# SEAME-pt/Team02-ObjectDetection

Measured on AMD Instinct MI355X. Metric: images/sec fwd+bwd MobileNetV2UNet 256x512 bs=32/GPU, higher is better.
Workload: dtype f32; 1 GPU; MobileNetV2UNet 10-class fwd+bwd+Adam, 256x512, bs=32/GPU (BASELINE configs[1]); model=MobileNetV2UNet, global_batch=32, parallelism=dp1, collectives=RCCL (torch.distributed nccl), optimizer=seg_amd.Adam (HIP, one launch)

## Files before the change

### include/segamd.h

```cpp
#ifndef SEGAMD_H
#define SEGAMD_H
#include <hip/hip_runtime.h>
#include <stdint.h>
#ifdef __cplusplus
extern "C" {
#endif



int seg_conv_igemm(const float* in, long ldin, int N, int H, int W, int Cin,
                   const float* wk, int ldk, const float* bias,
                   float* out, long ldout, int Ho, int Wo, int Cout,
                   int ks, int stride, int pad,
                   const float* add, long ldadd, float* stat, hipStream_t stream);
int seg_conv_igemm_act(const float* in, long ldin, int N, int H, int W, int Cin,
                       const float* wk, int ldk, const float* bias,
                       float* out, long ldout, int Ho, int Wo, int Cout,
                       int ks, int stride, int pad,
                       const float* add, long ldadd, float* stat, int act, float* work, int splits,
                       hipStream_t stream);
int seg_conv_igemm_bf16(const float* in, long ldin, int N, int H, int W, int Cin,
                        const float* wk, int ldk, const float* bias,
                        float* out, long ldout, int Ho, int Wo, int Cout,
                        int ks, int stride, int pad,
// ... 2 lines not shown
int seg_conv_igemm_f16(const float* in, long ldin, int N, int H, int W, int Cin,
                       const float* wk, int ldk, const float* bias,
                       float* out, long ldout, int Ho, int Wo, int Cout,
                       int ks, int stride, int pad,
                       const float* add, long ldadd, float* stat, int act, float* work, int splits,
                       hipStream_t stream);
int seg_conv_pw_row_tiles(long M);
int seg_conv_pw(const float* in, long ldin, long M, int K, const float* wk, int ldk, const float* bias,
                float* out, long ldout, int N, const float* add, long ldadd, float* stat,
                const float* in_scale, const float* in_shift, int in_act, hipStream_t stream);
int seg_conv_igemm_splits(long M, int Cout, int Cin, int ks);
int seg_conv_igemm_tiles(long M, int Cout);
int seg_conv_igemm_plan_b1(long M, int Cout, int Cin, int ks, int* out);
int seg_conv_igemm_act_ic(const float* in, long ldin, int N, int H, int W, int Cin, const float* wk, int ldk,
                          const float* bias, float* out, long ldout, int Ho, int Wo, int Cout, int ks, int stride,
                          int pad, const float* add, long ldadd, int act, float* work, int splits, int tile, unsigned* cnt,
                          hipStream_t stream);
int seg_conv_igemm_bf16_ic(const float* in, long ldin, int N, int H, int W, int Cin, const float* wk, int ldk,
                           const float* bias, float* out, long ldout, int Ho, int Wo, int Cout, int ks, int stride,
                           int pad, const float* add, long ldadd, int act, float* work, int splits, int tile, unsigned* cnt,
                           hipStream_t stream);
int seg_conv_igemm_f16_ic(const float* in, long ldin, int N, int H, int W, int Cin, const float* wk, int ldk,
                          const float* bias, float* out, long ldout, int Ho, int Wo, int Cout, int ks, int stride,
                          int pad, const float* add, long ldadd, int act, float* work, int splits, int tile, unsigned* cnt,
                          hipStream_t stream);

int seg_conv_igemm_bnout_ok(long M, int Cout, int bf16);
int seg_conv_igemm_bnout(const float* in, long ldin, int N, int H, int W, int Cin, const float* wk, int ldk,
                         float* out, long ldout, int Cout, int ks, const float* add, long ldadd,
                         const float* by, long ldby, const float* bscale, const float* bshift,
                         const float* bmean, int bact, float* bpart, hipStream_t stream);

int seg_igemm_force_tile(int t);
int seg_conv_igemm_tile(long M, int Cout);
int seg_conv_igemm_row_tiles(long M, int Cout, int* tile_rows);

int seg_pack_conv_weight(const float* w, float* wk, int Cout, int Cin, int ks, int ldk,
                         int mode, int kin_pad, hipStream_t stream);

int seg_conv_wgrad_splits(long M, int Cout, int Cin, int ks);
int seg_conv_wgrad_splits_bf16(long M, int Cout, int Cin, int ks);
int seg_conv_wgrad(const float* dy, long lddy, const float* x, long ldx,
                   int N, int H, int W, int Cin, int Ho, int Wo, int Cout,
                   int ks, int stride, int pad, float* part, int splits, hipStream_t stream);

int seg_conv_wgrad_bf16(const float* dy, long lddy, const float* x, long ldx,
                        int N, int H, int W, int Cin, int Ho, int Wo, int Cout,
                        int ks, int stride, int pad, float* part, int splits, hipStream_t stream);

int seg_conv_igemm_xf(const float* in, long ldin, int N, int H, int W, int Cin,
                      const float* wk, int ldk, const float* bias,
                      float* out, long ldout, int Ho, int Wo, int Cout,
                      int ks, int stride, int pad,
                      const float* add, long ldadd, float* stat, const float* in_scale, const float* in_shift,
                      int in_act, hipStream_t stream);
int seg_conv_igemm_bf16_xf(const float* in, long ldin, int N, int H, int W, int Cin,
                           const float* wk, int ldk, const float* bias,
                           float* out, long ldout, int Ho, int Wo, int Cout,
                           int ks, int stride, int pad,
                           const float* add, long ldadd, float* stat, const float* in_scale, const float* in_shift,
                           int in_act, hipStream_t stream);
int seg_conv_wgrad_xf(const float* dy, long lddy, const float* x, long ldx,
                      int N, int H, int W, int Cin, int Ho, int Wo, int Cout,
                      int ks, int stride, int pad, float* part, int splits,
                      const float* in_scale, const float* in_shift, int in_act, hipStream_t stream);
int seg_conv_wgrad_bf16_xf(const float* dy, long lddy, const float* x, long ldx,
                           int N, int H, int W, int Cin, int Ho, int Wo, int Cout,
                           int ks, int stride, int pad, float* part, int splits,
                           const float* in_scale, const float* in_shift, int in_act, hipStream_t stream);

int seg_conv_wgrad_reduce(const float* part, int splits, float* dw, int Cout, int Cin, int ks,
                          int mode, int accumulate, hipStream_t stream);

int seg_conv_wino_pick(int N, int H, int W, int Cin, int Cout);
int seg_conv_wino_tile_rows(void);
int seg_conv_wino_row_tiles(int N, int H, int W);
int seg_conv_wino(const float* in, long ldin, int N, int H, int W, int Cin, const float* wk, int ldk,
                  const float* bias, float* out, long ldout, int Cout, const float* add, long ldadd,
                  float* stat, float* work, hipStream_t stream);
int seg_conv_wino_fused(const float* in, long ldin, int N, int H, int W, int Cin, const float* wk, int ldk,
                        const float* bias, float* out, long ldout, int Cout, const float* add, long ldadd, float* stat,
                        hipStream_t stream);
int seg_conv_wino_fused_ok(int N, int H, int W, long ldin);
int seg_conv_wino_wgrad_pick(int N, int H, int W, int Cin, int Cout);
int seg_conv_wino_wgrad_splits(int N, int H, int W, int Cin, int Cout);
int seg_conv_wino_wgrad(const float* dy, long lddy, const float* x, long ldx, int N, int H, int W, int Cin,
                        int Cout, float* part, int splits, hipStream_t stream);
int seg_conv_wino_wgrad16_splits(int N, int H, int W, int Cin, int Cout);
int seg_conv_wino_wgrad16(const float* dy, long lddy, const float* x, long ldx, int N, int H, int W, int Cin,
                          int Cout, float* part, int splits, hipStream_t stream);
int seg_conv_wino_wgrad_reduce(float* part, int splits, float* dw, int Cout, int Cin, int Cin_pad,
                               int accumulate, hipStream_t stream);

int seg_conv_halo_ok(int N, int H, int W, int Cin, int Cout);
int seg_conv_halo_pick(int N, int H, int W, int Cin, int Cout);
int seg_conv_halo_row_tiles(int N, int H, int W);
int seg_conv_halo(const float* in, long ldin, int N, int H, int W, int Cin, const float* wk, int ldk,
                  const float* bias, float* out, long ldout, int Cout, const float* add, long ldadd,
                  float* stat, hipStream_t stream);

typedef struct seg_pack_job {
  const float* w;
  float* wk;
  int cout, cin, ks, ldk, mode, kin_pad;
  int blk0, nblk;
} seg_pack_job;
int seg_pack_batch(const void* jobs, int njobs, long nblocks, hipStream_t stream);

int seg_pack_dw_weight(const float* w, float* wk, int C, hipStream_t stream);
int seg_dw_fwd(const float* in, long ldin, int N, int H, int W, int C,
               const float* in_scale, const float* in_shift, int in_act, const float* wk,
               float* out, long ldout, int Ho, int Wo, int stride, hipStream_t stream);
int seg_dw_fwd_bias_act(const float* in, long ldin, int N, int H, int W, int C, const float* wk,
                        const float* bias, int act, float* out, long ldout, int Ho, int Wo, int stride,
                        hipStream_t stream);
int seg_dw_dgrad(const float* dy, long lddy, int N, int Ho, int Wo, int C, const float* wk,
                 float* dx, long lddx, int H, int W, int stride, int accumulate, hipStream_t stream);
long seg_dw_wgrad_blocks(int N, int Ho, int Wo, int C);
int seg_dw_wgrad(const float* dy, long lddy, const float* x, long ldx, int N, int H, int W, int C,
                 const float* in_scale, const float* in_shift, int in_act,
                 int Ho, int Wo, int stride, float* part, hipStream_t stream);

int seg_nchw_to_nhwc(const float* x, int N, int C, int H, int W, float* out, int ld, hipStream_t stream);

long seg_chan_workspace_floats(long M, int C);
int seg_bn_stats(const float* y, long ldy, long M, int C, const float* gamma, const float* beta,
                 float eps, float momentum, float* running_mean, float* running_var,
                 long long* num_batches_tracked, float* work,
                 float* mean, float* invstd, float* scale, float* shift, hipStream_t stream);
int seg_bn_stats_tiles(const float* part, int ntiles, int tile_rows, long M, int C, const float* gamma,
                       const float* beta, float eps, float momentum, float* running_mean, float* running_var,
                       long long* num_batches_tracked, float* mean, float* invstd, float* scale, float* shift,
                       hipStream_t stream);
long seg_bn_stats_tiles_work_floats(int ntiles, int C);
int seg_bn_stats_tiles_ws(const float* part, int ntiles, int tile_rows, long M, int C, const float* gamma,
                          const float* beta, float eps, float momentum, float* running_mean, float* running_var,
                          long long* num_batches_tracked, float* mean, float* invstd, float* scale, float* shift,
                          float* work, hipStream_t stream);
int seg_bn_eval_coef(const float* gamma, const float* beta, const float* running_mean,
                     const float* running_var, float eps, int C, float* scale, float* shift,
                     hipStream_t stream);
int seg_bn_apply(const float* y, long ldy, long M, int C, const float* scale, const float* shift,
                 int act, const float* res, long ldres, float* out, long ldout, hipStream_t stream);
int seg_bn_backward(const float* da, long ldda, const float* y, long ldy, long M, int C,
                    const float* gamma, const float* mean, const float* invstd,
                    const float* scale, const float* shift, int act,
                    float* dgamma, float* dbeta, float* work, float* dy, long lddy, hipStream_t stream);
int seg_bn_bwd_finalize_tiles(const float* part, int ntiles, long M, int C, const float* gamma,
                              const float* invstd, float* dgamma, float* dbeta, float* coef, hipStream_t stream);
int seg_bn_bwd_coef(const float* da, long ldda, const float* y, long ldy, long M, int C, const float* gamma,
                    const float* mean, const float* invstd, const float* scale, const float* shift, int act,
                    float* dgamma, float* dbeta, float* work, float* coef, hipStream_t stream);
int seg_bn_bwd_apply(const float* da, long ldda, const float* y, long ldy, long M, int C, const float* mean,
                     const float* scale, const float* shift, int act, const float* coef, float* dy, long lddy,
                     hipStream_t stream);
int seg_bn_eval_backward(const float* da, long ldda, const float* y, long ldy, long M, int C,
                         const float* scale, const float* shift, int act, float* dy, long lddy,
                         hipStream_t stream);
int seg_bn_frozen_backward(const float* da, long ldda, const float* y, long ldy, long M, int C,
                           const float* scale, const float* shift, const float* running_mean,
                           const float* running_var, float eps, int act, float* dgamma, float* dbeta,
                           float* work, float* dy, long lddy, hipStream_t stream);
int seg_colsum(const float* y, long ldy, long M, int C, float* work, float* out, int accumulate,
               hipStream_t stream);
int seg_add(const float* a, long lda, const float* b, long ldb, long M, int C, float* out, long ldout,
            hipStream_t stream);
// ... 271 lines not shown
```

### team02-objectdetection_amd/csrc/wino.hip

```cpp
#include "common.h"

#ifndef SEG_WINO_OUT_CSPLIT
#define SEG_WINO_OUT_CSPLIT 1
#endif

#ifndef SEG_WINO_OUT_QT
#define SEG_WINO_OUT_QT 4
#endif

namespace {

constexpr int kWinoQT = SEG_WINO_OUT_QT;
__device__ __attribute__((aligned(16))) float g_wzero4[4];

struct WinoArgs {
  const float* in; long ldin;
  const float* wk; int ldk;
  float* m;
  int N, H, W, Cin, Cout;
  int T, th, tw;
};

__device__ __forceinline__ void bt_row(int r, int& p0, int& p1, float& s0, float& s1) {
  p0 = r == 0 ? 0 : 1;
// ... 186 lines not shown
        for (int x = 0; x < 16; ++x) qv[x] = ld4(m + x * TC + (long)tile[q] * Cout + c);
        f32x4 r0[4], r1[4];
#pragma unroll
        for (int j = 0; j < 4; ++j) {
          r0[j] = qv[j] + qv[4 + j] + qv[8 + j];
          r1[j] = qv[4 + j] - qv[8 + j] - qv[12 + j];
        }
        y[q][0] = r0[0] + r0[1] + r0[2] + b;
        y[q][1] = r0[1] - r0[2] - r0[3] + b;
        y[q][2] = r1[0] + r1[1] + r1[2] + b;
        y[q][3] = r1[1] - r1[2] - r1[3] + b;
#pragma unroll
        for (int p = 0; p < 4; ++p) {
          if (add) y[q][p] += ld4(add + pix[q][p] * ldadd + c);
          st4(out + pix[q][p] * ldout + c, y[q][p]);
        }
      } else {
#pragma unroll
        for (int p = 0; p < 4; ++p) y[q][p] = f32x4{0.f, 0.f, 0.f, 0.f};
      }
    }
#if SEG_WINO_OUT_CSPLIT
    if (!stat) return;
#else
    if (!stat) continue;
#endif
#pragma unroll
    for (int pass = 0; pass < 2; ++pass) {
      f32x4 s = {0.f, 0.f, 0.f, 0.f};
      const f32x4 mu = pass ? bmean[cl] : f32x4{0.f, 0.f, 0.f, 0.f};
#pragma unroll
      for (int q = 0; q < QT; ++q)
        if (tok[q] && cok) {
#pragma unroll
          for (int p = 0; p < 4; ++p) {
            const f32x4 d = y[q][p] - mu;
            s += pass ? d * d : d;
          }
        }
#pragma unroll
      for (int o = 16; o < 64; o <<= 1)
#pragma unroll
        for (int j = 0; j < 4; ++j) s[j] += __shfl_xor(s[j], o, 64);
      if ((t & 63) < 16) red[wave][cl] = s;
      __syncthreads();
      if (t < 16) {
        const f32x4 tot = red[0][t] + red[1][t] + red[2][t] + red[3][t];
        const int cc = cgb + t * 4;
        if (pass == 0) bmean[t] = tot / cnt;
        if (cc < Cout) {
          float* dst = stat + ((long)blockIdx.x * 2 + pass) * Cout + cc;
#pragma unroll
          for (int j = 0; j < 4; ++j) dst[j] = tot[j];
        }
      }
      __syncthreads();
    }
  }
}

template <int BM, int BN, int WM, int WN, int NT = 256>
void launch_wino(const WinoArgs& a, hipStream_t s) {
  dim3 grid(seg_cdiv(a.T, BM) * seg_cdiv(a.Cout, BN), 1, 16);
  hipLaunchKernelGGL((wino_gemm_kernel<BM, BN, WM, WN, 32, NT>), grid, dim3(NT), 0, s, a);
}
#ifndef SEG_WINO_WIDE_MINBLK
#define SEG_WINO_WIDE_MINBLK 0
#endif
#ifndef SEG_WINO_WIDE
#define SEG_WINO_WIDE 256
#endif

struct WinoFusedArgs {
  const float* in; long ldin;
  const float* wk; int ldk;
  const float* bias;
  const float* add; long ldadd;
  float* out; long ldout;
  float* stat;
  int N, H, W, Cin, Cout;
  int T, th, tw;
  long in_elems;
  unsigned wk_bytes;
};

#ifndef SEG_WF_EXP
#define SEG_WF_EXP 0
#endif
constexpr int kFusedKC = 8;
constexpr int kFusedUR = kFusedKC + 4;
constexpr unsigned kFusedOOB = 0x80000000u;

__device__ __forceinline__ __amdgpu_buffer_rsrc_t seg_rsrc(const void* p, unsigned bytes) {
  const unsigned long v = (unsigned long)p;
  const unsigned lo = __builtin_amdgcn_readfirstlane((unsigned)v), hi = __builtin_amdgcn_readfirstlane((unsigned)(v >> 32));
  return __builtin_amdgcn_make_buffer_rsrc(reinterpret_cast<void*>(((unsigned long)hi << 32) | lo), 0,
                                           (int)__builtin_amdgcn_readfirstlane(bytes), 0x00020000);
}
__device__ __forceinline__ f32x4 seg_bld4(__amdgpu_buffer_rsrc_t r, unsigned off) {
  typedef unsigned u32x4 __attribute__((ext_vector_type(4)));
  return __builtin_bit_cast(f32x4, __builtin_amdgcn_raw_buffer_load_b128(r, off, 0, 0));
}

template <int WT>
__global__ __launch_bounds__(256) void wino_fused_kernel(WinoFusedArgs a) {
  constexpr int WN = 4 / WT, BT = 32 * WT, BC = 32 * WN;
  static_assert(WT == 2 || WT == 4, "a BN row tile (64 tiles) lies in one block");
  static_assert(16 * kWinoQT == 64, "wino_fused_kernel's BN row tile is 64 Winograd tiles");
  constexpr int USZ = 16 * BC * kFusedUR;
  constexpr int UPT = 16 * BC * (kFusedKC / 4) / 256;
  __shared__ __attribute__((aligned(16))) float Us[2 * USZ];
  __shared__ float red[4][32];

  const int tid = threadIdx.x, lane = tid & 63, wave = tid >> 6;
  const int wt = wave / WN, wn = wave % WN;
  const int row = lane & 31, h = lane >> 5;
  const int tiles_n = (a.Cout + BC - 1) / BC;
  const int lid = xcd_swizzle(blockIdx.x, gridDim.x);
  const int tn = lid % tiles_n, tm = lid / tiles_n;
  const int m0 = tm * BT, n0 = tn * BC;
  const int nfirst = m0 / (a.th * a.tw);
  const long boff = (long)nfirst * a.H * a.W * a.ldin;
  const __amdgpu_buffer_rsrc_t rin = seg_rsrc(a.in + boff, (unsigned)min((a.in_elems - boff) * 4, (long)kFusedOOB - 16));
  const __amdgpu_buffer_rsrc_t rwk = seg_rsrc(a.wk, a.wk_bytes);

  const int t = m0 + wt * 32 + row;
  const bool tok = t < a.T;
  unsigned pm = 0, pbase = 0;
  int opix = 0;
  {
    const int tt = tok ? t : 0;
    const int n = tt / (a.th * a.tw), r = tt - n * a.th * a.tw;
    const int ty = r / a.tw, tx = r - ty * a.tw;
    const int h0 = 2 * ty - 1, w0 = 2 * tx - 1;
#pragma unroll
    for (int p = 0; p < 4; ++p)
#pragma unroll
      for (int q = 0; q < 4; ++q)
        if (tok && (unsigned)(h0 + p) < (unsigned)a.H && (unsigned)(w0 + q) < (unsigned)a.W) pm |= 1u << (p * 4 + q);
    pbase = (unsigned)((((long)(n - nfirst) * a.H + h0) * a.W + w0) * a.ldin * 4) + 16u * h;
    opix = (n * a.H + 2 * ty) * a.W + 2 * tx;
  }
  const unsigned rstep = (unsigned)(a.W * a.ldin * 4), cstep = (unsigned)(a.ldin * 4);

  auto load_patch = [&](int c0, f32x4 (&d)[16]) {
    const bool cok = c0 + 4 * h < a.Cin;
    const unsigned b = pbase + 4u * c0;
#pragma unroll
    for (int p = 0; p < 4; ++p)
#pragma unroll
      for (int q = 0; q < 4; ++q) {
        const bool ok = cok && ((pm >> (p * 4 + q)) & 1u);
        d[p * 4 + q] = seg_bld4(rin, ok ? b + p * rstep + q * cstep : kFusedOOB);
      }
  };
  auto load_u = [&](int c0, f32x4 (&u)[UPT]) {
#pragma unroll
    for (int i = 0; i < UPT; ++i) {
      const int idx = tid + i * 256;
      const int xi = idx / (2 * BC), rem = idx - xi * (2 * BC);
      const int co = n0 + (rem >> 1), c = c0 + 4 * (rem & 1);
      const bool ok = co < a.Cout && c < a.Cin;
      u[i] = seg_bld4(rwk, ok ? (unsigned)((((long)xi * a.Cout + co) * a.ldk + c) * 4) : kFusedOOB);
    }
  };
  auto store_u = [&](float* dst, const f32x4 (&u)[UPT]) {
#pragma unroll
    for (int i = 0; i < UPT; ++i) {
      const int idx = tid + i * 256;
      const int xi = idx / (2 * BC), rem = idx - xi * (2 * BC);
      st4(dst + (xi * BC + (rem >> 1)) * kFusedUR + 4 * (rem & 1), u[i]);
    }
  };
  auto transform = [](f32x4 (&d)[16]) {
#pragma unroll
    for (int q = 0; q < 4; ++q) {
      const f32x4 d0 = d[q], d1 = d[4 + q], d2 = d[8 + q], d3 = d[12 + q];
      d[q] = d0 - d2;
      d[4 + q] = d1 + d2;
      d[8 + q] = d2 - d1;
      d[12 + q] = d1 - d3;
    }
#pragma unroll
    for (int r = 0; r < 4; ++r) {
      const f32x4 t0 = d[4 * r], t1 = d[4 * r + 1], t2 = d[4 * r + 2], t3 = d[4 * r + 3];
      d[4 * r] = t0 - t2;
      d[4 * r + 1] = t1 + t2;
      d[4 * r + 2] = t2 - t1;
      d[4 * r + 3] = t1 - t3;
    }
  };

  f32x16 acc[16];
#pragma unroll
  for (int x = 0; x < 16; ++x)
#pragma unroll
    for (int r = 0; r < 16; ++r) acc[x][r] = 0.f;

  const int nk = (a.Cin + kFusedKC - 1) / kFusedKC;
  const int urow = (wn * 32 + row) * kFusedUR + 4 * h;
  f32x4 d[16], ug[UPT];
  load_patch(0, d);
  load_u(0, ug);
  store_u(Us, ug);
  __syncthreads();
  for (int kc = 0; kc < nk; ++kc) {
    const bool more = kc + 1 < nk;
    f32x4 dn[16];
    if (more && !(SEG_WF_EXP & 1)) {
      load_patch((kc + 1) * kFusedKC, dn);
      load_u((kc + 1) * kFusedKC, ug);
    }
    if (SEG_WF_EXP & 1) {
#pragma unroll
      for (int q = 0; q < 16; ++q) dn[q] = d[q] * 0.5f;
    }
    if (!(SEG_WF_EXP & 2)) transform(d);
    const float* ub = Us + (kc & 1) * USZ + urow;
    f32x4 u[2][4];
#pragma unroll
    for (int j = 0; j < 4; ++j) u[0][j] = ld4(ub + j * BC * kFusedUR);
#pragma unroll
    for (int g = 0; g < 4; ++g) {
      if (g < 3) {
#pragma unroll
        for (int j = 0; j < 4; ++j) u[(g + 1) & 1][j] = ld4(ub + (4 * (g + 1) + j) * BC * kFusedUR);
      }
#pragma unroll
      for (int s2 = 0; s2 < 4; ++s2)
#pragma unroll
        for (int j = 0; j < 4; ++j)
          if (SEG_WF_EXP & 4)
            acc[4 * g + j][s2] += d[4 * g + j][s2] * u[g & 1][j][s2];
          else
            acc[4 * g + j] = __builtin_amdgcn_mfma_f32_32x32x2f32(d[4 * g + j][s2], u[g & 1][j][s2], acc[4 * g + j],
                                                                  0, 0, 0);
    }
    if (more) {
      store_u(Us + ((kc + 1) & 1) * USZ, ug);
#pragma unroll
      for (int q = 0; q < 16; ++q) d[q] = dn[q];
    }
    __syncthreads();
  }

  const int col = n0 + wn * 32 + row;
  const bool cok = col < a.Cout;
  const float b = (a.bias && cok) ? a.bias[col] : 0.f;
  auto tile_y = [&](int r, float (&y)[4]) {
    float q[16];
#pragma unroll
    for (int x = 0; x < 16; ++x) q[x] = acc[x][r];
    float r0[4], r1[4];
#pragma unroll
    for (int j = 0; j < 4; ++j) {
      r0[j] = q[j] + q[4 + j] + q[8 + j];
      r1[j] = q[4 + j] - q[8 + j] - q[12 + j];
    }
    y[0] = r0[0] + r0[1] + r0[2] + b;
    y[1] = r0[1] - r0[2] - r0[3] + b;
    y[2] = r1[0] + r1[1] + r1[2] + b;
    y[3] = r1[1] - r1[2] - r1[3] + b;
  };
  const int wbase = m0 + wt * 32 + 4 * h;
  float ssum = 0.f;
#pragma unroll
  for (int r = 0; r < 16; ++r) {
    const int tt = wbase + (r & 3) + 8 * (r >> 2);
    const long p0 = __shfl(opix, (r & 3) + 8 * (r >> 2) + 4 * h, 64);
    if (tt < a.T && cok) {
      float y[4];
      tile_y(r, y);
#pragma unroll
      for (int u = 0; u < 4; ++u) {
        const long pix = p0 + (u >> 1) * a.W + (u & 1);
        if (a.add) y[u] += a.add[pix * a.ldadd + col];
        a.out[pix * a.ldout + col] = y[u];
        ssum += y[u];
      }
    }
  }
  if (!a.stat) return;
  const int rtile = (m0 + (wt & ~1) * 32) / 64;
  const int ntile = min(64, a.T - rtile * 64);
  const int we = (wt & ~1) * WN + wn, wo = we + WN;
  float mean = 0.f;
#pragma unroll
  for (int pass = 0; pass < 2; ++pass) {
    float sv = ssum;
    if (pass) {
      sv = 0.f;
#pragma unroll
      for (int r = 0; r < 16; ++r) {
        const int tt = wbase + (r & 3) + 8 * (r >> 2);
        if (tt < a.T && cok) {
          float y[4];
          tile_y(r, y);
#pragma unroll
          for (int u = 0; u < 4; ++u) {
            const float dv = y[u] - mean;
            sv += dv * dv;
          }
        }
      }
    }
    sv += __shfl_xor(sv, 32, 64);
    if (h == 0) red[wave][row] = sv;
    __syncthreads();
    const float tot = red[we][row] + red[wo][row];
    if (pass == 0) mean = ntile > 0 ? tot / (4.f * (float)ntile) : 0.f;
    if ((wt & 1) == 0 && h == 0 && cok && ntile > 0) a.stat[((long)rtile * 2 + pass) * a.Cout + col] = tot;
    __syncthreads();
  }
}

struct WinoWgradArgs {
  const float* dy; long lddy;
  const float* x; long ldx;
  float* part;
  int N, H, W, Cin, Cout;
  int T, th, tw, kchunk;
};

__device__ __forceinline__ float arow(int i, int a) {
  return a == 0 ? (i == 3 ? 0.f : 1.f) : (i == 0 ? 0.f : (i == 2 || i == 3 ? -1.f : 1.f));
// ... 294 lines not shown
#pragma unroll
  for (int p = 0; p < 4; ++p) {
    float* slab = a.part + ((long)split * 16 + 4 * wave + p) * a.Cout * a.Cin;
#pragma unroll
    for (int ni = 0; ni < NI; ++ni) {
      const int col = n0 + ni * 32 + lrow;
      if (col >= a.Cin) continue;
#pragma unroll
      for (int mi = 0; mi < MI; ++mi)
#pragma unroll
        for (int e = 0; e < 16; ++e) {
          const int row = co0 + mi * 32 + (e & 3) + 8 * (e >> 2) + 4 * lh;
          if (row < a.Cout) slab[(long)row * a.Cin + col] = acc[p][mi][ni][e];
        }
    }
  }
}

__global__ __launch_bounds__(256) void wino_wgrad_fold_kernel(float* __restrict__ part, int splits, int L, long E4) {
  const long e = (long)blockIdx.x * 256 + threadIdx.x;
  if (e >= E4) return;
  const int s0 = blockIdx.y * L, s1 = min(splits, s0 + L);
  f32x4* p = reinterpret_cast<f32x4*>(part) + e;
  f32x4 acc = p[(long)s0 * E4];
#pragma unroll 8
  for (int s = s0 + 1; s < s1; ++s) acc += p[(long)s * E4];
  p[(long)s0 * E4] = acc;
}

__global__ __launch_bounds__(256) void wino_wgrad_reduce_kernel(const float* __restrict__ part, int splits, int stride,
                                                                int Cout, int Cin_pad, int Cin, float* __restrict__ dw,
                                                                int accumulate) {
  const long i = (long)blockIdx.x * 256 + threadIdx.x;
  if (i >= (long)Cout * Cin) return;
  const int co = (int)(i / Cin), ci = (int)(i - (long)co * Cin);
  const long plane = (long)Cout * Cin_pad, off = (long)co * Cin_pad + ci;
  float m[16];
#pragma unroll
  for (int x = 0; x < 16; ++x) m[x] = 0.f;
  for (int s = 0; s < splits; ++s) {
    const float* p = part + (long)s * stride * 16 * plane + off;
#pragma unroll
    for (int x = 0; x < 16; ++x) m[x] += p[x * plane];
  }
  float t[3][4];
#pragma unroll
  for (int j = 0; j < 4; ++j) {
    t[0][j] = m[j] + 0.5f * (m[4 + j] + m[8 + j]);
    t[1][j] = 0.5f * (m[4 + j] - m[8 + j]);
    t[2][j] = 0.5f * (m[4 + j] + m[8 + j]) + m[12 + j];
  }
  float* o = dw + i * 9;
#pragma unroll
  for (int y = 0; y < 3; ++y) {
    const float v[3] = {t[y][0] + 0.5f * (t[y][1] + t[y][2]), 0.5f * (t[y][1] - t[y][2]),
                        0.5f * (t[y][1] + t[y][2]) + t[y][3]};
#pragma unroll
    for (int x = 0; x < 3; ++x) o[y * 3 + x] = accumulate ? o[y * 3 + x] + v[x] : v[x];
  }
}

}

#ifndef SEG_WINO_FUSED
#define SEG_WINO_FUSED 1
#endif
static bool fused_fits(int N, int H, int W, long ldin) {
  const long tiles = (long)(H / 2) * (W / 2);
  const long imgs = std::min<long>(N, tiles > 0 ? 128 / tiles + 2 : N);
  return imgs * H * W * ldin * 4 < (long)kFusedOOB - 16;
}
SEG_API int seg_conv_wino_pick(int N, int H, int W, int Cin, int Cout) {
  if ((H & 1) || (W & 1) || (Cin & 3) || (Cout & 3) || N <= 0) return 0;
  if (Cin >= 256 && Cout >= 128) return 1;
  if (Cin >= 128 && Cout >= 128 && (Cout <= 2 * Cin || Cout >= 512)) return 1;
  const bool fits = fused_fits(N, H, W, Cin + 64);
  return (SEG_WINO_FUSED && fits && Cin >= 64 && (Cout >= 128 || (Cout >= 64 && Cin > 128 && Cin < 256))) ? 2 : 0;
}

SEG_API int seg_conv_wino_fused_ok(int N, int H, int W, long ldin) {
  return ((H & 1) || (W & 1) || N <= 0) ? 0 : (int)fused_fits(N, H, W, ldin);
}

SEG_API int seg_conv_wino_row_tiles(int N, int H, int W) {
  const long T = (long)N * (H / 2) * (W / 2);
  return (int)((T + 16 * kWinoQT - 1) / (16 * kWinoQT));
}

SEG_API int seg_conv_wino_tile_rows(void) { return 64 * kWinoQT; }

SEG_API int seg_conv_wino(const float* in, long ldin, int N, int H, int W, int Cin, const float* wk, int ldk,
                          const float* bias, float* out, long ldout, int Cout, const float* add, long ldadd,
                          float* stat, float* work, hipStream_t stream) {
  if ((H & 1) || (W & 1) || (Cin & 3) || (ldin & 3) || (ldk & 3) || ldk < Cin || (Cout & 3) || (ldout & 3) ||
      (add && (ldadd & 3)) || !work)
    return (int)hipErrorInvalidValue;
  WinoArgs a;
  a.in = in; a.ldin = ldin; a.wk = wk; a.ldk = ldk; a.m = work;
  a.N = N; a.H = H; a.W = W; a.Cin = Cin; a.Cout = Cout;
  a.th = H / 2; a.tw = W / 2; a.T = N * a.th * a.tw;
  if (a.T == 0) return 0;
  if (Cout >= SEG_WINO_WIDE && seg_cdiv(Cout, 256) * 2 == seg_cdiv(Cout, 128) &&
      (long)seg_cdiv(a.T, 128) * seg_cdiv(Cout, 256) * 16 >= SEG_WINO_WIDE_MINBLK)
    launch_wino<128, 256, 64, 64, 512>(a, stream);
  else if (Cout >= 128) launch_wino<128, 128, 64, 64>(a, stream);
  else launch_wino<128, 64, 64, 32>(a, stream);
  hipLaunchKernelGGL(wino_out_kernel, dim3(seg_cdiv(a.T, 16 * kWinoQT), SEG_WINO_OUT_CSPLIT ? seg_cdiv(Cout, 64) : 1), dim3(256), 0, stream, work, a.T, Cout, N, H, W, a.th,
                     a.tw, bias, add, ldadd, out, ldout, stat);
  SEG_RET_LAST();
}

SEG_API int seg_conv_wino_fused(const float* in, long ldin, int N, int H, int W, int Cin, const float* wk, int ldk,
                                const float* bias, float* out, long ldout, int Cout, const float* add, long ldadd,
                                float* stat, hipStream_t stream) {
  if ((H & 1) || (W & 1) || (Cin & 3) || (ldin & 3) || (ldk & 3) || ldk < Cin || (Cout & 3) || (add && ldadd < Cout) ||
      ldout < Cout)
    return (int)hipErrorInvalidValue;
  WinoFusedArgs a;
  a.in = in; a.ldin = ldin; a.wk = wk; a.ldk = ldk; a.bias = bias; a.add = add; a.ldadd = ldadd;
  a.out = out; a.ldout = ldout; a.stat = stat;
  a.N = N; a.H = H; a.W = W; a.Cin = Cin; a.Cout = Cout;
  a.th = H / 2; a.tw = W / 2; a.T = N * a.th * a.tw;
  if (a.T == 0) return 0;
  const long wk_bytes = 16L * Cout * ldk * 4;
  if (!fused_fits(N, H, W, ldin) || wk_bytes >= (long)kFusedOOB) return (int)hipErrorInvalidValue;
  a.in_elems = ((long)N * H * W - 1) * ldin + Cin;
  a.wk_bytes = (unsigned)wk_bytes;
  hipLaunchKernelGGL(wino_fused_kernel<4>, dim3(seg_cdiv(a.T, 128) * seg_cdiv(Cout, 32)), dim3(256), 0, stream, a);
  SEG_RET_LAST();
}

SEG_API int seg_conv_wino_wgrad_pick(int N, int H, int W, int Cin, int Cout) {
  if ((H & 1) || (W & 1) || (Cin & 3) || (Cout & 3)) return 0;
  return (Cin >= 32 && Cout >= 32) ? 2 : 0;
}

#ifndef SEG_WW16_WIDE
#define SEG_WW16_WIDE 128
#endif
static int wgrad16_tile(int Cin, int Cout) { return (Cin >= SEG_WW16_WIDE && Cout >= SEG_WW16_WIDE) ? 64 : 32; }

SEG_API int seg_conv_wino_wgrad16_splits(int N, int H, int W, int Cin, int Cout) {
  const long T = (long)N * (H / 2) * (W / 2);
  const int b = wgrad16_tile(Cin, Cout);
  const long tiles = (long)seg_cdiv(Cout, b) * seg_cdiv(Cin, b);
  const long slots = b == 64 ? 256 : 512;
  const double u = b == 64 ? 490.0 : 300.0, slab_ns = 16.0 * Cout * Cin * 4 * 2 / 4000.0;
  const long smax = std::max<long>(1, std::min<long>(1024, T / 64));
  long best = 1;
  double best_t = 0;
  for (long sp = 1; sp <= smax; ++sp) {
    const long chunk = seg_cdiv(seg_cdiv(T, sp), (long)WBK) * WBK;
    const long used = seg_cdiv(T, chunk);
    const double t = (double)seg_cdiv(sp * tiles, slots) * chunk * u + sp * slab_ns;
    if (used == sp && (sp == 1 || t < best_t)) best = sp, best_t = t;
  }
  return (int)best;
}

SEG_API int seg_conv_wino_wgrad_splits(int N, int H, int W, int Cin, int Cout) {
  const long T = (long)N * (H / 2) * (W / 2);
  const int bm = Cout >= 128 ? 128 : (Cout >= 64 ? 64 : 32);
  const int bn = bm == 32 ? 128 : (Cin >= 128 ? 128 : 64);
  const long tiles = 16L * seg_cdiv(Cout, bm) * seg_cdiv(Cin, bn);
  long splits = (2048 + tiles - 1) / tiles;
  splits = std::min(splits, std::max<long>(1, T / 128));
  return (int)std::max<long>(1, std::min<long>(splits, 1024));
}

SEG_API int seg_conv_wino_wgrad(const float* dy, long lddy, const float* x, long ldx, int N, int H, int W, int Cin,
                                int Cout, float* part, int splits, hipStream_t stream) {
  if ((H & 1) || (W & 1) || (Cin & 3) || (Cout & 3) || (lddy & 3) || (ldx & 3) || splits < 1)
    return (int)hipErrorInvalidValue;
  WinoWgradArgs a;
  a.dy = dy; a.lddy = lddy; a.x = x; a.ldx = ldx; a.part = part;
  a.N = N; a.H = H; a.W = W; a.Cin = Cin; a.Cout = Cout;
  a.th = H / 2; a.tw = W / 2; a.T = N * a.th * a.tw;
  a.kchunk = seg_cdiv(seg_cdiv(a.T, splits), WBK) * WBK;
  const int bm = Cout >= 128 ? 128 : (Cout >= 64 ? 64 : 32);
  const int bn = bm == 32 ? 128 : (Cin >= 128 ? 128 : 64);
  dim3 grid(seg_cdiv(Cout, bm) * seg_cdiv(Cin, bn) * splits, 1, 16);
  if (bm == 128 && bn == 128) hipLaunchKernelGGL((wino_wgrad_kernel<128, 128, 64, 64>), grid, dim3(256), 0, stream, a);
  else if (bm == 128) hipLaunchKernelGGL((wino_wgrad_kernel<128, 64, 64, 32>), grid, dim3(256), 0, stream, a);
  else if (bm == 64 && bn == 128) hipLaunchKernelGGL((wino_wgrad_kernel<64, 128, 32, 64>), grid, dim3(256), 0, stream, a);
  else if (bm == 64) hipLaunchKernelGGL((wino_wgrad_kernel<64, 64, 32, 32>), grid, dim3(256), 0, stream, a);
  else hipLaunchKernelGGL((wino_wgrad_kernel<32, 128, 32, 32>), grid, dim3(256), 0, stream, a);
  SEG_RET_LAST();
}

SEG_API int seg_conv_wino_wgrad16(const float* dy, long lddy, const float* x, long ldx, int N, int H, int W, int Cin,
                                  int Cout, float* part, int splits, hipStream_t stream) {
  if ((H & 1) || (W & 1) || (Cin & 3) || (Cout & 3) || (lddy & 3) || (ldx & 3) || splits < 1)
    return (int)hipErrorInvalidValue;
  WinoWgradArgs a;
  a.dy = dy; a.lddy = lddy; a.x = x; a.ldx = ldx; a.part = part;
  a.N = N; a.H = H; a.W = W; a.Cin = Cin; a.Cout = Cout;
  a.th = H / 2; a.tw = W / 2; a.T = N * a.th * a.tw;
  a.kchunk = seg_cdiv(seg_cdiv(a.T, splits), WBK) * WBK;
  if (a.T == 0) return 0;
  const long span = (2L * (seg_cdiv(a.kchunk, a.tw) + 1) + 2) * W * std::max(ldx, lddy) * 4;
  if (span >= (long)kFusedOOB - 16) return seg_conv_wino_wgrad(dy, lddy, x, ldx, N, H, W, Cin, Cout, part, splits, stream);
  const int b = wgrad16_tile(Cin, Cout);
  const dim3 grid(seg_cdiv(Cout, b) * seg_cdiv(Cin, b) * splits);
  if (b == 64) hipLaunchKernelGGL((wino_wgrad16_kernel<64, 64, 8>), grid, dim3(256), 0, stream, a);
  else hipLaunchKernelGGL((wino_wgrad16_kernel<32, 32, 16>), grid, dim3(256), 0, stream, a);
  SEG_RET_LAST();
}

SEG_API int seg_conv_wino_wgrad_reduce(float* part, int splits, float* dw, int Cout, int Cin, int Cin_pad,
                                       int accumulate, hipStream_t stream) {
  if (Cin_pad < Cin || (Cin_pad & 3) || splits < 1) return (int)hipErrorInvalidValue;
// ... 13 lines not shown
```

### team02-objectdetection_amd/seg_amd/_lib.py

```python
from __future__ import annotations

import ctypes
import os
import threading

from .build import LIB_PATH, source_hash

_V = ctypes.c_void_p
_I = ctypes.c_int
_L = ctypes.c_long
_F = ctypes.c_float

PROTOTYPES = {
    "seg_conv_igemm": (_I, [_V, _L, _I, _I, _I, _I, _V, _I, _V, _V, _L, _I, _I, _I, _I, _I, _I, _V, _L, _V, _V]),
    "seg_conv_igemm_act": (_I, [_V, _L, _I, _I, _I, _I, _V, _I, _V, _V, _L, _I, _I, _I, _I, _I, _I, _V, _L, _V, _I,
                                _V, _I, _V]),
    "seg_conv_igemm_bf16": (_I, [_V, _L, _I, _I, _I, _I, _V, _I, _V, _V, _L, _I, _I, _I, _I, _I, _I, _V, _L, _V, _I,
                                 _V, _I, _V]),
    "seg_conv_igemm_f16": (_I, [_V, _L, _I, _I, _I, _I, _V, _I, _V, _V, _L, _I, _I, _I, _I, _I, _I, _V, _L, _V, _I,
                                _V, _I, _V]),
    "seg_conv_igemm_splits": (_I, [_L, _I, _I, _I]),
    "seg_igemm_force_tile": (_I, [_I]),
    "seg_conv_igemm_tile": (_I, [_L, _I]),
    "seg_conv_halo_ok": (_I, [_I, _I, _I, _I, _I]),
    "seg_conv_halo_pick": (_I, [_I, _I, _I, _I, _I]),
    "seg_conv_halo_row_tiles": (_I, [_I, _I, _I]),
    "seg_conv_halo": (_I, [_V, _L, _I, _I, _I, _I, _V, _I, _V, _V, _L, _I, _V, _L, _V, _V]),
    "seg_conv_wino_pick": (_I, [_I, _I, _I, _I, _I]),
    "seg_conv_wino_row_tiles": (_I, [_I, _I, _I]),
    "seg_conv_wino_tile_rows": (_I, []),
    "seg_conv_wino": (_I, [_V, _L, _I, _I, _I, _I, _V, _I, _V, _V, _L, _I, _V, _L, _V, _V, _V]),
    "seg_conv_wino_fused": (_I, [_V, _L, _I, _I, _I, _I, _V, _I, _V, _V, _L, _I, _V, _L, _V, _V]),
    "seg_conv_wino_fused_ok": (_I, [_I, _I, _I, _L]),
    "seg_conv_wino_wgrad_pick": (_I, [_I, _I, _I, _I, _I]),
    "seg_conv_wino_wgrad_splits": (_I, [_I, _I, _I, _I, _I]),
    "seg_conv_wino_wgrad": (_I, [_V, _L, _V, _L, _I, _I, _I, _I, _I, _V, _I, _V]),
    "seg_conv_wino_wgrad16_splits": (_I, [_I, _I, _I, _I, _I]),
    "seg_conv_wino_wgrad16": (_I, [_V, _L, _V, _L, _I, _I, _I, _I, _I, _V, _I, _V]),
    "seg_conv_wino_wgrad_reduce": (_I, [_V, _I, _V, _I, _I, _I, _I, _V]),
    "seg_pack_batch": (_I, [_V, _I, _L, _V]),
    "seg_conv_igemm_row_tiles": (_I, [_L, _I, _V]),
    "seg_pack_conv_weight": (_I, [_V, _V, _I, _I, _I, _I, _I, _I, _V]),
    "seg_conv_wgrad_splits": (_I, [_L, _I, _I, _I]),
    "seg_conv_wgrad_splits_bf16": (_I, [_L, _I, _I, _I]),
    "seg_conv_wgrad": (_I, [_V, _L, _V, _L, _I, _I, _I, _I, _I, _I, _I, _I, _I, _I, _V, _I, _V]),
    "seg_conv_wgrad_bf16": (_I, [_V, _L, _V, _L, _I, _I, _I, _I, _I, _I, _I, _I, _I, _I, _V, _I, _V]),
    "seg_conv_wgrad_reduce": (_I, [_V, _I, _V, _I, _I, _I, _I, _I, _V]),
    "seg_pack_dw_weight": (_I, [_V, _V, _I, _V]),
    "seg_dw_fwd": (_I, [_V, _L, _I, _I, _I, _I, _V, _V, _I, _V, _V, _L, _I, _I, _I, _V]),
    "seg_dw_fwd_bias_act": (_I, [_V, _L, _I, _I, _I, _I, _V, _V, _I, _V, _L, _I, _I, _I, _V]),
    "seg_dw_dgrad": (_I, [_V, _L, _I, _I, _I, _I, _V, _V, _L, _I, _I, _I, _I, _V]),
    "seg_dw_wgrad_blocks": (_L, [_I, _I, _I, _I]),
    "seg_dw_wgrad": (_I, [_V, _L, _V, _L, _I, _I, _I, _I, _V, _V, _I, _I, _I, _I, _V, _V]),
    "seg_nchw_to_nhwc": (_I, [_V, _I, _I, _I, _I, _V, _I, _V]),
    "seg_chan_workspace_floats": (_L, [_L, _I]),
    "seg_bn_stats": (_I, [_V, _L, _L, _I, _V, _V, _F, _F, _V, _V, _V, _V, _V, _V, _V, _V, _V]),
    "seg_bn_stats_tiles": (_I, [_V, _I, _I, _L, _I, _V, _V, _F, _F, _V, _V, _V, _V, _V, _V, _V, _V]),
    "seg_bn_stats_tiles_ws": (_I, [_V, _I, _I, _L, _I, _V, _V, _F, _F, _V, _V, _V, _V, _V, _V, _V, _V, _V]),
    "seg_bn_stats_tiles_work_floats": (_L, [_I, _I]),
    "seg_bn_eval_coef": (_I, [_V, _V, _V, _V, _F, _I, _V, _V, _V]),
    "seg_bn_apply": (_I, [_V, _L, _L, _I, _V, _V, _I, _V, _L, _V, _L, _V]),
    "seg_bn_backward": (_I, [_V, _L, _V, _L, _L, _I, _V, _V, _V, _V, _V, _I, _V, _V, _V, _V, _L, _V]),
    "seg_bn_eval_backward": (_I, [_V, _L, _V, _L, _L, _I, _V, _V, _I, _V, _L, _V]),
    "seg_bn_frozen_backward": (_I, [_V, _L, _V, _L, _L, _I, _V, _V, _V, _V, _F, _I, _V, _V, _V, _V, _L, _V]),
    "seg_colsum": (_I, [_V, _L, _L, _I, _V, _V, _I, _V]),
    "seg_add": (_I, [_V, _L, _V, _L, _L, _I, _V, _L, _V]),
    "seg_upsample_fwd": (_I, [_V, _L, _I, _I, _I, _I, _V, _L, _I, _I, _I, _V]),
    "seg_upsample_bwd": (_I, [_V, _L, _I, _I, _I, _I, _I, _V, _L, _I, _I, _I, _I, _V]),
    "seg_upsample_to_nchw": (_I, [_V, _L, _I, _I, _I, _I, _V, _I, _I, _I, _V]),
    "seg_maxpool2_fwd": (_I, [_V, _L, _I, _I, _I, _I, _V, _L, _V]),
    "seg_maxpool2_bwd": (_I, [_V, _L, _V, _L, _I, _I, _I, _I, _V, _L, _I, _V]),
    "seg_ce_workspace_floats": (_L, [_L]),
    "seg_ce_upsample_loss": (_I, [_V, _L, _I, _I, _I, _I, _V, _I, _I, _I, _V, _V, _V]),
    "seg_ce_upsample_grad": (_I, [_V, _L, _I, _I, _I, _I, _V, _I, _I, _I, _V, _V, _V, _L, _V]),
    "seg_ce_upsample_eval": (_I, [_V, _L, _I, _I, _I, _I, _V, _I, _I, _I, _V, _V, _V, _V]),
    "seg_cew_workspace_floats": (_L, [_L]),
    "seg_cew_upsample_loss": (_I, [_V, _L, _I, _I, _I, _I, _V, _I, _I, _I, _V, _F, _I, _V, _V, _V]),
    "seg_cew_upsample_grad": (_I, [_V, _L, _I, _I, _I, _I, _V, _I, _I, _I, _V, _F, _V, _V, _V, _L, _V]),
    "seg_cew_upsample_eval": (_I, [_V, _L, _I, _I, _I, _I, _V, _I, _I, _I, _V, _F, _I, _V, _V, _V, _V]),
    "seg_sl_workspace_floats": (_L, [_L]),
    "seg_sl_upsample_loss": (_I, [_V, _L, _I, _I, _I, _I, _V, _I, _I, _I, _V, _F, _F, _F, _F, _F, _V, _V, _V, _V]),
    "seg_sl_upsample_eval": (_I, [_V, _L, _I, _I, _I, _I, _V, _I, _I, _I, _V, _F, _F, _F, _F, _F, _V, _V, _V, _V,
                                  _V]),
    "seg_sl_upsample_grad": (_I, [_V, _L, _I, _I, _I, _I, _V, _I, _I, _I, _V, _F, _F, _F, _F, _V, _V, _V, _V, _L,
                                  _V]),
    "seg_bn_fold_batch": (_I, [_V, _I, _L, _V]),
    "seg_preprocess_bgr": (_I, [_V, _I, _I, _I, _L, _V, _I, _I, _I, _F, _F, _F, _F, _F, _F, _V]),
    "seg_argmax_nearest": (_I, [_V, _L, _I, _I, _I, _I, _I, _I, _V, _I, _I, _V]),
    "seg_resize_u8": (_I, [_V, _I, _I, _I, _L, _V, _I, _I, _I, _V, _V]),
    "seg_augment": (_I, [_V, _V, _I, _I, _I, _V, _F, _F, _F, _F, _F, _F, _V, _V, _V]),
    "seg_adam_step": (_I, [_V, _V, _I, _I, _F, _F, _F, _F, _V]),
    "seg_adam_step_skip": (_I, [_V, _V, _I, _I, _F, _F, _F, _F, _V, _V]),
    "seg_adamw_step": (_I, [_V, _V, _I, _I, _F, _F, _F, _F, _V, _V, _V]),
    "seg_grad_norm_workspace_floats": (_L, [_I]),
    "seg_grad_sumsq": (_I, [_V, _V, _I, _I, _F, _V, _V, _V]),
    "seg_grad_scale": (_I, [_V, _V, _I, _I, _V, _V]),
    "seg_tape_fn_index": (_I, [ctypes.c_char_p]),
    "seg_tape_fn_nargs": (_I, [_I]),
    "seg_tape_create": (_I, [_V, _I, _V, _L, _I, _V]),
    "seg_tape_destroy": (_I, [_V]),
    "seg_tape_set_arg": (_I, [_V, _L, _L]),
    "seg_tape_timing": (_I, [_V, _V, _I, _I]),
    "seg_tape_elapsed": (_I, [_V, _V]),
    "seg_tape_timeline": (_I, [_V, _I, _V]),
    "seg_tape_run": (_I, [_V, _I, _V, _V, _V]),
    "seg_set_combine_spin": (_I, [_I]),
    "seg_build_hash": (_I, [ctypes.c_char_p, _I]),
    "seg_conv_igemm2_plan": (_I, [_L, _I, _I, _I, _V]),
    "seg_conv_pw_row_tiles": (_I, [_L]),
    "seg_conv_pw": (_I, [_V, _L, _L, _I, _V, _I, _V, _V, _L, _I, _V, _L, _V, _V, _V, _I, _V]),
    "seg_conv_igemm2_bf16io": (_I, [_V, _L, _I, _I, _I, _I, _V, _I, _V, _V, _L, _I, _I, _V, _L, _V, _V, _V]),
    "seg_igemm2_force_tile": (_I, [_I]),
    "seg_igemm2_tune": (_I, [_I, _I]),
    "seg_conv_wgrad2_ok": (_I, [_I, _I, _I, _I, _I]),
    "seg_conv_wgrad2_blocks": (_I, [_I, _I, _I]),
    "seg_conv_wgrad2_bf16io": (_I, [_V, _L, _V, _L, _I, _I, _I, _I, _I, _V, _V]),
# ... 106 lines not shown
```

Measured before the change: 2038 images/s.

## Stage Winograd fused input halo into LDS via direct global-to-LDS DMA

Adds a halo-staging form of the fused Winograd forward kernel. Each block cooperatively DMAs its input patch region, including the halo, into double-buffered dynamic LDS using global_load_lds, with a swizzle and a zero row for out-of-bounds reads. Threads then read their 4x4 patches from LDS instead of issuing overlapping global loads. It is selected by default when the staging size fits, which raises dynamic LDS use and may reduce occupancy while adding waitcnt/sync costs.

```diff
diff --git a/include/segamd.h b/include/segamd.h
--- a/include/segamd.h
+++ b/include/segamd.h
@@ -108,6 +108,9 @@
                         const float* bias, float* out, long ldout, int Cout, const float* add, long ldadd, float* stat,
                         hipStream_t stream);
 int seg_conv_wino_fused_ok(int N, int H, int W, long ldin);
+int seg_conv_wino_fused_halo_stage(int N, int H, int W);
+int seg_conv_wino_fused_form(int N, int H, int W);
+int seg_wino_fused_force_form(int form);
 int seg_conv_wino_wgrad_pick(int N, int H, int W, int Cin, int Cout);
 int seg_conv_wino_wgrad_splits(int N, int H, int W, int Cin, int Cout);
 int seg_conv_wino_wgrad(const float* dy, long lddy, const float* x, long ldx, int N, int H, int W, int Cin,
diff --git a/team02-objectdetection_amd/csrc/wino.hip b/team02-objectdetection_amd/csrc/wino.hip
--- a/team02-objectdetection_amd/csrc/wino.hip
+++ b/team02-objectdetection_amd/csrc/wino.hip
@@ -292,6 +292,7 @@
   int T, th, tw;
   long in_elems;
   unsigned wk_bytes;
+  unsigned hstage;
 };
 
 #ifndef SEG_WF_EXP
@@ -312,7 +313,15 @@
   return __builtin_bit_cast(f32x4, __builtin_amdgcn_raw_buffer_load_b128(r, off, 0, 0));
 }
 
-template <int WT>
+constexpr unsigned kHaloStageMax = 54 * 1024;
+__device__ __attribute__((aligned(16))) unsigned g_wino_zero_row[4];
+__device__ __forceinline__ void wino_dma16(const void* src, char* lds) {
+  __builtin_amdgcn_global_load_lds((const __attribute__((address_space(1))) void*)src,
+                                   (__attribute__((address_space(3))) void*)lds, 16, 0, 0);
+}
+__device__ __forceinline__ int halo_swz(int x) { return x ^ ((x >> 4) & 1); }
+
+template <int WT, bool HALO>
 __global__ __launch_bounds__(256) void wino_fused_kernel(WinoFusedArgs a) {
   constexpr int WN = 4 / WT, BT = 32 * WT, BC = 32 * WN;
   static_assert(WT == 2 || WT == 4, "a BN row tile (64 tiles) lies in one block");
@@ -321,6 +330,7 @@
   constexpr int UPT = 16 * BC * (kFusedKC / 4) / 256;
   __shared__ __attribute__((aligned(16))) float Us[2 * USZ];
   __shared__ float red[4][32];
+  extern __shared__ __attribute__((aligned(1024))) char halo_stage[];
 
   const int tid = threadIdx.x, lane = tid & 63, wave = tid >> 6;
   const int wt = wave / WN, wn = wave % WN;
@@ -353,6 +363,60 @@
   }
   const unsigned rstep = (unsigned)(a.W * a.ldin * 4), cstep = (unsigned)(a.ldin * 4);
 
+  int hrow0 = 0, hcol0 = 0, hcols = 0, hnblk = 1, hpieces = 0;
+  int hcolL = 0;
+  long hsrc = 0;
+  unsigned hrd = 0, hrdq[4] = {0, 0, 0, 0};
+  if constexpr (HALO) {
+    const int tpi = a.th * a.tw;
+    const int r0 = m0 - nfirst * tpi, r1 = min(m0 + BT, a.T) - 1 - nfirst * tpi;
+    const int ty0 = r0 / a.tw, ty1 = r1 / a.tw;
+    const int tx0 = ty0 == ty1 ? r0 - ty0 * a.tw : 0, tx1 = ty0 == ty1 ? r1 - ty1 * a.tw : a.tw - 1;
+    hrow0 = 2 * ty0 - 1;
+    hcol0 = 2 * tx0 - 1;
+    hcols = 2 * (tx1 - tx0) + 4;
+    hnblk = (hcols + 31) >> 5;
+    hpieces = (2 * (ty1 - ty0) + 4) * hnblk;
+    hcolL = hcol0 + halo_swz(lane & 31);
+    hsrc = (((long)nfirst * a.H + hrow0) * a.W + hcolL) * a.ldin + 4 * h;
+    const int rl = (tok ? t : m0) - nfirst * tpi;
+    const int ty = rl / a.tw, tx = rl - ty * a.tw;
+    hrd = (unsigned)(2 * (ty - ty0) * hnblk) * 1024u + 512u * h;
+#pragma unroll
+    for (int q = 0; q < 4; ++q) {
+      const int c = 2 * tx - 1 - hcol0 + q;
+      hrdq[q] = (unsigned)(c >> 5) * 1024u + 16u * halo_swz(c & 31);
+    }
+  }
+  const void* zrow = nullptr;
+  if constexpr (HALO) {
+    zrow = g_wino_zero_row;
+    asm volatile("" : "+s"(zrow));
+  }
+  auto stage_halo = [&](int c0, char* sb) {
+    const int uw = __builtin_amdgcn_readfirstlane(wave);
+    const bool cok = c0 + 4 * h < a.Cin;
+    int r = 0, b = uw;
+    for (int j = uw; j < hpieces; j += 4) {
+      while (b >= hnblk) {
+        b -= hnblk;
+        ++r;
+      }
+      const int ih = hrow0 + r, iw = hcolL + 32 * b;
+      const bool ok = cok && (unsigned)ih < (unsigned)a.H && (unsigned)iw < (unsigned)a.W && iw < hcol0 + hcols;
+      const float* src = a.in + hsrc + ((long)r * a.W + 32 * b) * a.ldin + c0;
+      wino_dma16(ok ? (const void*)src : zrow, sb + j * 1024);
+      b += 4;
+    }
+  };
+  auto read_patch = [&](const char* sb, f32x4 (&d)[16]) {
+    const unsigned rs = (unsigned)hnblk * 1024u;
+#pragma unroll
+    for (int p = 0; p < 4; ++p)
+#pragma unroll
+      for (int q = 0; q < 4; ++q) d[p * 4 + q] = ld4(reinterpret_cast<const float*>(sb + hrd + p * rs + hrdq[q]));
+  };
+
   auto load_patch = [&](int c0, f32x4 (&d)[16]) {
     const bool cok = c0 + 4 * h < a.Cin;
     const unsigned b = pbase + 4u * c0;
@@ -410,18 +474,27 @@
   const int nk = (a.Cin + kFusedKC - 1) / kFusedKC;
   const int urow = (wn * 32 + row) * kFusedUR + 4 * h;
   f32x4 d[16], ug[UPT];
-  load_patch(0, d);
+  if constexpr (HALO)
+    stage_halo(0, halo_stage);
+  else
+    load_patch(0, d);
   load_u(0, ug);
   store_u(Us, ug);
+  if constexpr (HALO) __builtin_amdgcn_s_waitcnt(0x0F70);
   __syncthreads();
   for (int kc = 0; kc < nk; ++kc) {
     const bool more = kc + 1 < nk;
     f32x4 dn[16];
     if (more && !(SEG_WF_EXP & 1)) {
-      load_patch((kc + 1) * kFusedKC, dn);
+      if constexpr (HALO)
+        stage_halo((kc + 1) * kFusedKC, halo_stage + ((kc + 1) & 1) * a.hstage);
+      else
+        load_patch((kc + 1) * kFusedKC, dn);
       load_u((kc + 1) * kFusedKC, ug);
     }
-    if (SEG_WF_EXP & 1) {
+    if constexpr (HALO) {
+      read_patch(halo_stage + ((SEG_WF_EXP & 1) ? 0 : kc & 1) * a.hstage, d);
+    } else if (SEG_WF_EXP & 1) {
 #pragma unroll
       for (int q = 0; q < 16; ++q) dn[q] = d[q] * 0.5f;
     }
@@ -448,9 +521,12 @@
     }
     if (more) {
       store_u(Us + ((kc + 1) & 1) * USZ, ug);
-#pragma unroll
-      for (int q = 0; q < 16; ++q) d[q] = dn[q];
-    }
+      if constexpr (!HALO) {
+#pragma unroll
+        for (int q = 0; q < 16; ++q) d[q] = dn[q];
+      }
+    }
+    if constexpr (HALO) __builtin_amdgcn_s_waitcnt(0x0F70);
     __syncthreads();
   }
 
@@ -911,6 +987,34 @@
   return ((H & 1) || (W & 1) || N <= 0) ? 0 : (int)fused_fits(N, H, W, ldin);
 }
 
+static unsigned wino_fused_halo_stage(int N, int H, int W) {
+  if ((H & 1) || (W & 1) || N <= 0 || H < 2 || W < 2) return 0;
+  const int th = H / 2, tw = W / 2;
+  const long tpi = (long)th * tw;
+  if (N > 1 && tpi % 128 != 0) return 0;
+  int rows;
+  if (tw % 128 == 0) rows = 1;
+  else if (128 % tw == 0 && tpi % 128 == 0) rows = 128 / tw;
+  else rows = std::min(th, (tw + 126) / tw + 1);
+  const long cols = rows == 1 ? std::min(W + 2, 258) : W + 2;
+  const long bytes = (2L * rows + 2) * ((cols + 31) / 32) * 1024;
+  return bytes <= (long)kHaloStageMax ? (unsigned)bytes : 0u;
+}
+SEG_API int seg_conv_wino_fused_halo_stage(int N, int H, int W) { return (int)wino_fused_halo_stage(N, H, W); }
+
+static int g_wino_fused_forced_form = -1;
+SEG_API int seg_wino_fused_force_form(int form) {
+  if (form < -1 || form > 1) return (int)hipErrorInvalidValue;
+  g_wino_fused_forced_form = form;
+  return 0;
+}
+SEG_API int seg_conv_wino_fused_form(int N, int H, int W) {
+  const bool ok = wino_fused_halo_stage(N, H, W) != 0;
+  if (g_wino_fused_forced_form == 0) return 0;
+  if (g_wino_fused_forced_form == 1) return ok ? 1 : -1;
+  return ok ? 1 : 0;
+}
+
 SEG_API int seg_conv_wino_row_tiles(int N, int H, int W) {
   const long T = (long)N * (H / 2) * (W / 2);
   return (int)((T + 16 * kWinoQT - 1) / (16 * kWinoQT));
@@ -955,7 +1059,25 @@
   if (!fused_fits(N, H, W, ldin) || wk_bytes >= (long)kFusedOOB) return (int)hipErrorInvalidValue;
   a.in_elems = ((long)N * H * W - 1) * ldin + Cin;
   a.wk_bytes = (unsigned)wk_bytes;
-  hipLaunchKernelGGL(wino_fused_kernel<4>, dim3(seg_cdiv(a.T, 128) * seg_cdiv(Cout, 32)), dim3(256), 0, stream, a);
+  a.hstage = 0;
+  const dim3 grid(seg_cdiv(a.T, 128) * seg_cdiv(Cout, 32));
+  const int form = seg_conv_wino_fused_form(N, H, W);
+  if (form < 0) return (int)hipErrorInvalidValue;
+  if (form == 1) {
+    static bool raised[64];
+    int dev = 0;
+    if (hipGetDevice(&dev) != hipSuccess || dev < 0 || dev >= 64) return (int)hipErrorInvalidValue;
+    if (!raised[dev]) {
+      const hipError_t e = hipFuncSetAttribute(reinterpret_cast<const void*>(&wino_fused_kernel<4, true>),
+                                               hipFuncAttributeMaxDynamicSharedMemorySize, 2 * (int)kHaloStageMax);
+      if (e != hipSuccess) return (int)e;
+      raised[dev] = true;
+    }
+    a.hstage = wino_fused_halo_stage(N, H, W);
+    hipLaunchKernelGGL((wino_fused_kernel<4, true>), grid, dim3(256), 2 * a.hstage, stream, a);
+  } else {
+    hipLaunchKernelGGL((wino_fused_kernel<4, false>), grid, dim3(256), 0, stream, a);
+  }
   SEG_RET_LAST();
 }
 
diff --git a/team02-objectdetection_amd/seg_amd/_lib.py b/team02-objectdetection_amd/seg_amd/_lib.py
--- a/team02-objectdetection_amd/seg_amd/_lib.py
+++ b/team02-objectdetection_amd/seg_amd/_lib.py
@@ -32,6 +32,9 @@
     "seg_conv_wino": (_I, [_V, _L, _I, _I, _I, _I, _V, _I, _V, _V, _L, _I, _V, _L, _V, _V, _V]),
     "seg_conv_wino_fused": (_I, [_V, _L, _I, _I, _I, _I, _V, _I, _V, _V, _L, _I, _V, _L, _V, _V]),
     "seg_conv_wino_fused_ok": (_I, [_I, _I, _I, _L]),
+    "seg_conv_wino_fused_halo_stage": (_I, [_I, _I, _I]),
+    "seg_conv_wino_fused_form": (_I, [_I, _I, _I]),
+    "seg_wino_fused_force_form": (_I, [_I]),
     "seg_conv_wino_wgrad_pick": (_I, [_I, _I, _I, _I, _I]),
     "seg_conv_wino_wgrad_splits": (_I, [_I, _I, _I, _I, _I]),
     "seg_conv_wino_wgrad": (_I, [_V, _L, _V, _L, _I, _I, _I, _I, _I, _V, _I, _V]),
```

Result: no change. 2057 images/s, median of 6 (+1.0%).
